# dusk-network/jubjub-schnorr

Hardware: AMD Instinct MI355X
Metric: Schnorr verifications/sec (higher is better)
Workload: dtype u32 limbs (29-bit), u64 accumulators

## Files before the change

### jubjub_schnorr_amd/csrc/ed29.h

```cpp
#pragma once
#include "fq29.h"

namespace jjs {

using fe_t = fe<1, 5>;

struct ext_pt {
    fe_n x, y, z, t;
};
struct niels_pt {
    fe_t ypx, ymx, z, t2d;
};

JJS_HD fe_n fe_n_one() { return fq_as<1, 2>(fq_one()); }
JJS_HD fe_n fe_n_zero() { return fq_as<1, 2>(fq_zero()); }

JJS_HD ext_pt ext_identity() {
    ext_pt p;
    p.x = fe_n_zero(); p.y = fe_n_one(); p.z = fe_n_one(); p.t = fe_n_zero();
    return p;
}
JJS_HD ext_pt ext_from_affine(const fe_n& u, const fe_n& v) {
    ext_pt p;
    p.x = u; p.y = v; p.z = fe_n_one(); p.t = fq_mul(u, v);
// ... 30 lines not shown
    ext_pt r;
    r.x = fq_mul_hot(e, f);
    r.z = fq_mul_hot(f, h);
    r.y = fq_mul_hot(h, g);
    if (need_t) r.t = fq_mul_hot(g, e); else r.t = fe_n_zero();
    return r;
}

JJS_HD ext_pt ext_add_niels(const ext_pt& p, const niels_pt& n, bool neg, bool need_t) {
    fe_t n_ymx = fq_select(neg, n.ypx, n.ymx);
    fe_t n_ypx = fq_select(neg, n.ymx, n.ypx);
    auto n_t2d = fq_select(neg, fq_neg(n.t2d), fq_as<2, 6>(n.t2d));
    fe_n a = fq_mul_hot(fq_sub(p.y, p.x), n_ymx);
    fe_n b = fq_mul_hot(fq_add(p.y, p.x), n_ypx);
    fe_n c = fq_mul_hot(p.t, n_t2d);
    auto d = fq_dbl(fq_mul_hot(p.z, n.z));
    auto e = fq_sub(b, a);
    auto f = fq_norm(fq_sub(d, c));
    auto g = fq_add(d, c);
    auto h = fq_norm(fq_add(b, a));
    ext_pt r;
    r.x = fq_mul_hot(e, f);
    r.z = fq_mul_hot(f, g);
    r.y = fq_mul_hot(g, h);
    if (need_t) r.t = fq_mul_hot(h, e); else r.t = fe_n_zero();
    return r;
}
JJS_HD ext_pt ext_add_affine_niels_signed(const ext_pt& p, const fe_t& n_ypx, const fe_t& n_ymx, const fe_t& n_t2d, bool neg,
                                          bool need_t) {
    fe_t s_ymx = fq_select(neg, n_ypx, n_ymx);
    fe_t s_ypx = fq_select(neg, n_ymx, n_ypx);
    auto s_t2d = fq_select(neg, fq_neg(n_t2d), fq_as<2, 6>(n_t2d));
    fe_n a = fq_mul_hot(fq_sub(p.y, p.x), s_ymx);
    fe_n b = fq_mul_hot(fq_add(p.y, p.x), s_ypx);
    fe_n c = fq_mul_hot(p.t, s_t2d);
    auto d = fq_dbl(p.z);
    auto e = fq_sub(b, a);
    auto f = fq_norm(fq_sub(d, c));
    auto g = fq_add(d, c);
    auto h = fq_norm(fq_add(b, a));
    ext_pt r;
    r.x = fq_mul_hot(e, f);
    r.z = fq_mul_hot(f, g);
    r.y = fq_mul_hot(g, h);
    if (need_t) r.t = fq_mul_hot(h, e); else r.t = fe_n_zero();
    return r;
}

JJS_HD ext_pt ext_add_affine_niels(const ext_pt& p, const fe_t& n_ypx, const fe_t& n_ymx, const fe_t& n_t2d,
                                   bool need_t) {
    return ext_add_affine_niels_signed(p, n_ypx, n_ymx, n_t2d, false, need_t);
}

JJS_HD bool ext_is_identity(const ext_pt& p) { return fq_is_zero(p.x) && fq_eq(p.y, p.z); }

JJS_HD bool affine_on_curve(const fe_n& u, const fe_n& v) {
    fe_n u2 = fq_sqr(u), v2 = fq_sqr(v);
    auto lhs = fq_sub(v2, u2);
    auto rhs = fq_norm(fq_add(fq_mul(fq_mul(u2, v2), fe_from_const<1, 1>(JJS_D)), fq_one()));
    return fq_eq(lhs, rhs);
}
JJS_HD bool affine_is_identity(const fe_n& u, const fe_n& v) { return fq_is_zero(u) && fq_eq(v, fq_one()); }

JJS_HD bool ext_eq_affine(const ext_pt& p, const fe_n& u, const fe_n& v) {
    return fq_eq(p.x, fq_mul(u, p.z)) && fq_eq(p.y, fq_mul(v, p.z));
}

}
```

### jubjub_schnorr_amd/csrc/fq29.h

```cpp
#pragma once
#include <stdint.h>

#if defined(__HIPCC__)
#include <hip/hip_runtime.h>
#define JJS_HD __host__ __device__ __forceinline__
#define JJS_CALL __host__ __device__ __attribute__((noinline))
#if defined(__HIP_DEVICE_COMPILE__)
#define JJS_CONST __constant__ const
#else
#define JJS_CONST static const
#endif
#else
#define JJS_HD inline __attribute__((always_inline))
#define JJS_CALL __attribute__((noinline))
#define JJS_CONST static const
#endif

namespace jjs {

#include "jjs_constants.inc"
#include "mont_asm.inc"

constexpr uint32_t MASK29 = 0x1fffffffu;

// ... 61 lines not shown
    for (int i = 0; i < 9; ++i) r.l[i] = a.l[i] + b.l[i];
    return r;
}
template <int L, int A>
JJS_HD fe<2 * L, 2 * A> fq_dbl(const fe<L, A>& a) {
    fe<2 * L, 2 * A> r;
#pragma unroll
    for (int i = 0; i < 9; ++i) r.l[i] = a.l[i] << 1;
    return r;
}
template <int La, int Aa, int Ab>
JJS_HD fe<La + 2, Aa + Ab + 1> fq_sub(const fe<La, Aa>& a, const fe<1, Ab>& b) {
    fe<La + 2, Aa + Ab + 1> r;
#pragma unroll
    for (int i = 0; i < 9; ++i) r.l[i] = a.l[i] + (subpad29(Ab + 1, i) - b.l[i]);
    return r;
}
template <int Ab>
JJS_HD fe<2, Ab + 1> fq_neg(const fe<1, Ab>& b) {
    fe<2, Ab + 1> r;
#pragma unroll
    for (int i = 0; i < 9; ++i) r.l[i] = subpad29(Ab + 1, i) - b.l[i];
    return r;
}
template <int L, int A>
JJS_HD fe<1, A> fq_norm(const fe<L, A>& a) {
    fe<1, A> r;
    uint32_t carry = 0;
#pragma unroll
    for (int i = 0; i < 8; ++i) {
        uint32_t t = a.l[i] + carry;
        r.l[i] = t & MASK29;
        carry = t >> 29;
    }
    r.l[8] = a.l[8] + carry;
    return r;
}
template <int A>
JJS_HD fe_n fq_reduce(const fe<1, A>& a) {
    static_assert(A <= 4, "fq_reduce handles values below 4q");
    fe_n t;
    int32_t borrow = 0;
#pragma unroll
    for (int i = 0; i < 9; ++i) {
        int32_t d = (int32_t)a.l[i] - (int32_t)kq29(2, i) + borrow;
        t.l[i] = (uint32_t)d & MASK29;
        borrow = d >> 29;
        if (i == 8) t.l[8] = (uint32_t)d;
    }
    bool neg = borrow < 0;
    fe_n r;
#pragma unroll
    for (int i = 0; i < 9; ++i) r.l[i] = neg ? a.l[i] : t.l[i];
    return r;
}
template <int L, int A>
JJS_HD fe<L, A> fq_select(bool c, const fe<L, A>& a, const fe<L, A>& b) {
    fe<L, A> r;
#pragma unroll
    for (int i = 0; i < 9; ++i) r.l[i] = c ? a.l[i] : b.l[i];
    return r;
}

JJS_HD int64_t mont_ashr29(int64_t v) {
    return v >> 29;
}

JJS_HD raw9 mont_mul_body(const uint32_t* a, const uint32_t* b) {
    int64_t m[9];
    raw9 r;
    int64_t acc = 0;
#pragma unroll
    for (int k = 0; k < 9; ++k) {
#pragma unroll
        for (int i = 0; i <= k; ++i) acc += (int64_t)((uint64_t)a[i] * b[k - i]);
#pragma unroll
        for (int i = 0; i < k; ++i) acc -= m[i] * (int64_t)q29(k - i);
        if (k < 8) {
            m[k] = acc & (int64_t)MASK29;
            acc = mont_ashr29(acc);
        } else {
            m[8] = (acc & (int64_t)MASK29) - ((int64_t)1 << 29);
            acc = mont_ashr29(acc - m[8]);
        }
    }
#pragma unroll
    for (int k = 9; k < 17; ++k) {
#pragma unroll
        for (int i = k - 8; i < 9; ++i) acc += (int64_t)((uint64_t)a[i] * b[k - i]);
#pragma unroll
        for (int i = k - 8; i < 9; ++i) acc -= m[i] * (int64_t)q29(k - i);
        r.l[k - 9] = (uint32_t)(acc & (int64_t)MASK29);
        acc = mont_ashr29(acc);
    }
    r.l[8] = (uint32_t)acc;
    return r;
}
JJS_HD raw9 mont_sqr_body(const uint32_t* a) {
    int64_t m[9];
    uint32_t a2[9];
#pragma unroll
    for (int i = 0; i < 9; ++i) a2[i] = a[i] << 1;
    raw9 r;
    int64_t acc = 0;
#pragma unroll
    for (int k = 0; k < 17; ++k) {
// ... 233 lines not shown
    fe_c r;
#pragma unroll
    for (int i = 0; i < 9; ++i) {
        int bit = 29 * i, w = bit >> 5, sh = bit & 31;
        uint64_t v = a.w[w];
        if (w + 1 < 8) v |= (uint64_t)a.w[w + 1] << 32;
        r.l[i] = (uint32_t)(v >> sh) & MASK29;
    }
    return r;
}
JJS_HD fe_n fq_from_words(const words8& a) { return fq_mul(words_to_limbs(a), fe_from_const<1, 1>(JJS_R2)); }

template <int L, int A>
JJS_HD fe_c fq_canon_limbs(const fe<L, A>& a) {
    fe_c one = fq_zero();
    one.l[0] = 1;
    fe_n y = fq_mul(fq_norm(a), one);
    bool is_q = true;
#pragma unroll
    for (int i = 0; i < 9; ++i) is_q = is_q && (y.l[i] == q29(i));
    fe_c r;
#pragma unroll
    for (int i = 0; i < 9; ++i) r.l[i] = is_q ? 0u : y.l[i];
    return r;
}
template <int L, int A>
JJS_HD words8 fq_to_words(const fe<L, A>& a) {
    fe_c c = fq_canon_limbs(a);
    words8 o;
#pragma unroll
    for (int w = 0; w < 8; ++w) {
        int bit = 32 * w, i = bit / 29, sh = bit - 29 * i;
        uint64_t v = (uint64_t)c.l[i] >> sh;
        int have = 29 - sh;
        v |= (uint64_t)c.l[i + 1] << have;
        if (have + 29 < 32 && i + 2 < 9) v |= (uint64_t)c.l[i + 2] << (have + 29);
        o.w[w] = (uint32_t)v;
    }
    return o;
}
template <int L, int A>
JJS_HD bool fq_is_zero(const fe<L, A>& a) {
    fe_c c = fq_canon_limbs(a);
    uint32_t x = 0;
#pragma unroll
    for (int i = 0; i < 9; ++i) x |= c.l[i];
    return x == 0;
}
template <int La, int Aa, int Ab>
JJS_HD bool fq_eq(const fe<La, Aa>& a, const fe<1, Ab>& b) {
    return fq_is_zero(fq_sub(a, b));
}

JJS_HD fe_n fq_pow_schedule(const fe_n& a, const uint32_t (*sched)[2], int steps, int trailing) {
    fe_n a2 = fq_sqr(a);
    fe_n a3 = fq_mul(a2, a), a5 = fq_mul(a3, a2), a7 = fq_mul(a5, a2);
    fe_n e = a;
    for (int st = 0; st < steps; ++st) {
        const uint32_t nsq = sched[st][0], dg = sched[st][1];
        if (st != 0)
            for (uint32_t j = 0; j < nsq; ++j) e = fq_sqr(e);
        const fe_n m = fq_select(dg == 1, a, fq_select(dg == 3, a3, fq_select(dg == 5, a5, a7)));
        e = (st == 0) ? m : fq_mul(e, m);
    }
    for (int j = 0; j < trailing; ++j) e = fq_sqr(e);
    return e;
}
}
```

### jubjub_schnorr_amd/csrc/jjs_constants.inc

```
#define JJS_MAX_HASH_INPUTS 16
#define JJS_Q29_0 0x00000001u
#define JJS_Q29_1 0x1ffffff8u
#define JJS_Q29_2 0x1f96ffbfu
#define JJS_Q29_3 0x1b4805ffu
#define JJS_Q29_4 0x1d80553bu
#define JJS_Q29_5 0x0c0404d0u
#define JJS_Q29_6 0x1520cce7u
#define JJS_Q29_7 0x0a6533afu
#define JJS_Q29_8 0x0073eda7u
JJS_CONST uint32_t JJS_Q_WORDS[8] = {0x00000001u, 0xffffffffu, 0xfffe5bfeu, 0x53bda402u, 0x09a1d805u, 0x3339d808u, 0x299d7d48u, 0x73eda753u};
JJS_CONST uint32_t JJS_QM2_WORDS[8] = {0xffffffffu, 0xfffffffeu, 0xfffe5bfeu, 0x53bda402u, 0x09a1d805u, 0x3339d808u, 0x299d7d48u, 0x73eda753u};
JJS_CONST uint32_t JJS_FR_WORDS[8] = {0xd6f72cb7u, 0xd0970e5eu, 0xccc81082u, 0xa6682093u, 0x01343b00u, 0x06673b01u, 0x6533afa9u, 0x0e7db4eau};
JJS_CONST uint32_t JJS_FR_R2_WORDS[8] = {0x95e57731u, 0x67719aa4u, 0x9ce3fc26u, 0x51b0cef0u, 0xc026e9a5u, 0x69dab7fau, 0x8d127688u, 0x04f6547bu};
#define JJS_FR_INV32 0xef788ef9u
JJS_CONST uint32_t JJS_R2[9] = {0x0a71b3c0u, 0x1d32207eu, 0x1663d999u, 0x1c5abc93u, 0x03b58c44u, 0x0be37438u, 0x0829f771u, 0x1660139eu, 0x0027fd91u};
JJS_CONST uint32_t JJS_ONE[9] = {0x1fffffbau, 0x0000022fu, 0x1cb61180u, 0x0a4e5c00u, 0x0ee8b1a2u, 0x16e6aedfu, 0x1907f8bbu, 0x0853ddf7u, 0x004d043fu};
JJS_CONST uint32_t JJS_D[9] = {0x0e9ed5e8u, 0x12245679u, 0x002d9f52u, 0x03bb3367u, 0x0d9bfb3du, 0x18ebb3ccu, 0x1c29ceccu, 0x0a7b6020u, 0x0020d725u};
JJS_CONST uint32_t JJS_D2[9] = {0x1d3dabd0u, 0x0448acf2u, 0x005b3ea5u, 0x077666ceu, 0x1b37f67au, 0x11d76798u, 0x18539d99u, 0x14f6c041u, 0x0041ae4au};
JJS_CONST uint32_t JJS_G[2][9] = {{0x0f8e352bu, 0x0d898cfcu, 0x1acf8b86u, 0x11cbaed5u, 0x11f53f06u, 0x1e102b0eu, 0x1a54d9c6u, 0x143eceffu, 0x006815d6u}, {0x1ffffb09u, 0x000027b7u, 0x09503dc0u, 0x0d6a3610u, 0x07d8d3d7u, 0x180c16bcu, 0x1a26af41u, 0x038c62dfu, 0x006f1642u}};
JJS_CONST uint32_t JJS_GN[2][9] = {{0x187d023du, 0x137e7289u, 0x0690434eu, 0x1f76361du, 0x00cee7a6u, 0x0f6ffe89u, 0x0eae76dcu, 0x0b002f63u, 0x001b3c2eu}, {0x0d19dfe5u, 0x1ba2bfe4u, 0x0aa87077u, 0x0a3c12aeu, 0x0f209d38u, 0x03331d80u, 0x05e964c7u, 0x046d436du, 0x00027722u}};
JJS_CONST uint32_t JJS_DOUBLE_TAG_WORDS[8] = {0x4844424cu, 0x4a4a5343u, 0x00000000u, 0x00000000u, 0x00000000u, 0x00000000u, 0x00000000u, 0x00000000u};
JJS_CONST uint32_t JJS_SPONGE_TAG[JJS_MAX_HASH_INPUTS + 1][9] = {
  {0x00000000u, 0x00000000u, 0x00000000u, 0x00000000u, 0x00000000u, 0x00000000u, 0x00000000u, 0x00000000u, 0x00000000u},
  {0x0505ee08u, 0x1a263c20u, 0x0be84b8bu, 0x14a02c49u, 0x01c71b32u, 0x0119871du, 0x0e158ab3u, 0x1ae4f29eu, 0x002534dfu},
  {0x1b0be909u, 0x1f0bd4a7u, 0x15c76ef6u, 0x19aa6651u, 0x03d277dau, 0x02c51eb8u, 0x131e6edfu, 0x1c823839u, 0x0028ae1cu},
  {0x0fc46418u, 0x0273db7eu, 0x16529079u, 0x104dd318u, 0x168e8637u, 0x026f5725u, 0x1c808eacu, 0x029e0e17u, 0x003fedbdu},
  {0x0357c163u, 0x10043808u, 0x19bdf7a6u, 0x0d30d38fu, 0x12e5297bu, 0x1c58dc5fu, 0x0ba83205u, 0x06d45679u, 0x00090830u},
  {0x0262554eu, 0x06977c58u, 0x1cc4c932u, 0x13bcc122u, 0x0d7d7321u, 0x16c6f8cdu, 0x0c42072du, 0x0a7ba9d5u, 0x00467f10u},
  {0x16ed364au, 0x0b0ae88eu, 0x1bd377f9u, 0x1bebcca6u, 0x0fbf0111u, 0x0eacca90u, 0x174be582u, 0x0d8cb0dfu, 0x006048a8u},
  {0x1648d83cu, 0x1c96a336u, 0x13f93121u, 0x0404c2c5u, 0x12088053u, 0x05063ca4u, 0x1387a958u, 0x0e2ca8b5u, 0x000dc63bu},
  {0x1f8df888u, 0x05a7ef5au, 0x1e8dea4fu, 0x04cf9c40u, 0x03a338cdu, 0x11ce25feu, 0x08f757fcu, 0x197c5746u, 0x00448b3du},
  {0x18861d85u, 0x0bfc90f3u, 0x01a0c7f1u, 0x0b8f8540u, 0x061d8364u, 0x17492b24u, 0x1f89fbceu, 0x03e0f6e4u, 0x002d13cau},
  {0x0f24fc1du, 0x17584430u, 0x197f7236u, 0x1bad9229u, 0x17ce7252u, 0x12745987u, 0x119f85a5u, 0x0365f792u, 0x00419641u},
  {0x0ad4ee1du, 0x1c33dd77u, 0x03cea63au, 0x0090b229u, 0x1eff0500u, 0x1ae3d4a9u, 0x0e58224eu, 0x1ba57ecau, 0x00131c30u},
  {0x0047e885u, 0x12b591deu, 0x09f50887u, 0x0c3877f6u, 0x01adcabbu, 0x00dcbf79u, 0x0ac6f554u, 0x0bcc64deu, 0x0062115cu},
  {0x18868630u, 0x0c3e88d9u, 0x0d12f54du, 0x062083b4u, 0x00efbe4eu, 0x1c915ba8u, 0x11f90d73u, 0x1200490cu, 0x00205cd9u},
  {0x109c52e0u, 0x100352e0u, 0x0d1863ecu, 0x0f9203ccu, 0x08db7deau, 0x1ea7d49cu, 0x0641cbbeu, 0x1693107au, 0x00056607u},
  {0x07380761u, 0x0379c563u, 0x10c89db4u, 0x0924fcebu, 0x0cf29ce1u, 0x1bfecb19u, 0x1a3ca913u, 0x12d81574u, 0x0008852cu},
  {0x0137f8a1u, 0x135b43b9u, 0x1a25c48fu, 0x04e620e0u, 0x0f670a49u, 0x190a832du, 0x1c3afc44u, 0x0c7a93dbu, 0x0026b4abu},
};
JJS_CONST uint32_t JJS_PAIR_L1[2][9] = {{0x1632f828u, 0x1cd998edu, 0x06ef42eau, 0x18522084u, 0x12362748u, 0x02a698c9u, 0x1b29c579u, 0x021b0691u, 0x003c41f3u}, {0x1b06fde4u, 0x137cdc5cu, 0x1714b9b2u, 0x065d7f7du, 0x140f3e68u, 0x08fb5d4bu, 0x18ad857au, 0x02b255c2u, 0x005ac97bu}};
JJS_CONST uint32_t JJS_PAIR_NEG_L2[9] = {0x0ec609f6u, 0x0fa98aa5u, 0x012a02e2u, 0x17e06bfeu, 0x14bb44c6u, 0x0c66138cu, 0x166a4edbu, 0x0ffd0b0au, 0x0050cfe0u};
JJS_CONST uint32_t JJS_PAIR_B[9] = {0x002c2b67u, 0x1e9ea4c8u, 0x07b6263fu, 0x1afbd911u, 0x133cdbc5u, 0x16559828u, 0x1a61d3c3u, 0x10975a2au, 0x00520471u};
JJS_CONST uint32_t JJS_PAIR_EXP_WORDS[8] = {0xe0000000u, 0xdfffffffu, 0x5fffcb7fu, 0xaa77b480u, 0x01343b00u, 0x06673b01u, 0x6533afa9u, 0x0e7db4eau};
#define JJS_PAIR_SW_STEPS 57
#define JJS_PAIR_SW_TRAILING 29
JJS_CONST uint32_t JJS_PAIR_SW[JJS_PAIR_SW_STEPS][2] = {{3, 7}, {5, 7}, {2, 3}, {3, 3}, {3, 3}, {2, 1}, {5, 7}, {4, 5}, {4, 3}, {5, 5}, {4, 3}, {5, 7}, {4, 5}, {3, 7}, {3, 5}, {2, 1}, {3, 1}, {7, 3}, {4, 3}, {5, 7}, {5, 7}, {3, 3}, {8, 1}, {8, 1}, {4, 3}, {2, 1}, {7, 7}, {3, 3}, {11, 5}, {4, 5}, {5, 7}, {4, 7}, {3, 5}, {3, 5}, {3, 1}, {11, 5}, {3, 7}, {3, 7}, {3, 7}, {3, 7}, {2, 3}, {5, 5}, {3, 5}, {3, 7}, {3, 7}, {2, 3}, {4, 7}, {3, 7}, {3, 7}, {3, 7}, {3, 7}, {3, 7}, {3, 7}, {3, 7}, {3, 7}, {3, 7}, {2, 3}};
#define JJS_INV_SW_STEPS 68
#define JJS_INV_SW_TRAILING 0
JJS_CONST uint32_t JJS_INV_SW[JJS_INV_SW_STEPS][2] = {{3, 7}, {5, 7}, {2, 3}, {3, 3}, {3, 3}, {2, 1}, {5, 7}, {4, 5}, {4, 3}, {5, 5}, {4, 3}, {5, 7}, {4, 5}, {3, 7}, {3, 5}, {2, 1}, {3, 1}, {7, 3}, {4, 3}, {5, 7}, {5, 7}, {3, 3}, {8, 1}, {8, 1}, {4, 3}, {2, 1}, {7, 7}, {3, 3}, {11, 5}, {4, 5}, {5, 7}, {4, 7}, {3, 5}, {3, 5}, {3, 1}, {11, 5}, {3, 7}, {3, 7}, {3, 7}, {3, 7}, {2, 3}, {5, 5}, {3, 5}, {3, 7}, {3, 7}, {2, 3}, {4, 7}, {3, 7}, {3, 7}, {3, 7}, {3, 7}, {3, 7}, {3, 7}, {3, 7}, {3, 7}, {3, 7}, {3, 5}, {3, 7}, {3, 7}, {3, 7}, {3, 7}, {3, 7}, {3, 7}, {3, 7}, {3, 7}, {3, 7}, {3, 7}, {1, 1}};
#define JJS_SQRT_SW_STEPS 57
#define JJS_SQRT_SW_TRAILING 0
JJS_CONST uint32_t JJS_SQRT_SW[JJS_SQRT_SW_STEPS][2] = {{3, 7}, {5, 7}, {2, 3}, {3, 3}, {3, 3}, {2, 1}, {5, 7}, {4, 5}, {4, 3}, {5, 5}, {4, 3}, {5, 7}, {4, 5}, {3, 7}, {3, 5}, {2, 1}, {3, 1}, {7, 3}, {4, 3}, {5, 7}, {5, 7}, {3, 3}, {8, 1}, {8, 1}, {4, 3}, {2, 1}, {7, 7}, {3, 3}, {11, 5}, {4, 5}, {5, 7}, {4, 7}, {3, 5}, {3, 5}, {3, 1}, {11, 5}, {3, 7}, {3, 7}, {3, 7}, {3, 7}, {2, 3}, {5, 5}, {3, 5}, {3, 7}, {3, 7}, {2, 3}, {4, 7}, {3, 7}, {3, 7}, {3, 7}, {3, 7}, {3, 7}, {3, 7}, {3, 7}, {3, 7}, {3, 7}, {1, 1}};
JJS_CONST uint32_t JJS_DLOG_BASES[7][9] = {{0x1e643334u, 0x16481b3cu, 0x1b429d12u, 0x177f9dadu, 0x144a8d18u, 0x0d45bdd8u, 0x04734720u, 0x08d7bfb9u, 0x0036d431u}, {0x015b5931u, 0x170bf111u, 0x0fdc692cu, 0x1da57375u, 0x1cd8fb0cu, 0x082b2e9eu, 0x11dae58du, 0x1c3e92cdu, 0x007386deu}, {0x046746cau, 0x011b8fe2u, 0x1ba33a6du, 0x176e1524u, 0x09d99e75u, 0x154d7d8eu, 0x00d23d31u, 0x1df2d37eu, 0x000963afu}, {0x1e643334u, 0x16481b3cu, 0x1b429d12u, 0x177f9dadu, 0x144a8d18u, 0x0d45bdd8u, 0x04734720u, 0x08d7bfb9u, 0x0036d431u}, {0x065b9ba7u, 0x16d68576u, 0x182b2c2au, 0x14d5af02u, 0x07140888u, 0x1362f1d7u, 0x08c77bb2u, 0x1cb1a9c5u, 0x00094bf1u}, {0x1abc62ceu, 0x0fbddb01u, 0x140b0090u, 0x03bc5521u, 0x11f8af58u, 0x1881ae47u, 0x11d5d43eu, 0x0a2d9980u, 0x005fe400u}, {0x04fbdc84u, 0x10c8e2ffu, 0x041d8af4u, 0x1a3da377u, 0x19ceef70u, 0x002b6e41u, 0x0034a007u, 0x1c185b28u, 0x0007ee60u}};
#define JJS_DLOG_HASH_MULT 1u
#define JJS_DLOG_HASH_SHIFT 0
JJS_CONST uint32_t JJS_ROOT_OF_UNITY[9] = {0x01c8cd27u, 0x158d8d27u, 0x19006c0du, 0x09177006u, 0x1b40635eu, 0x01d0b1cau, 0x0d517805u, 0x04859aa2u, 0x002c4064u};
JJS_CONST uint32_t JJS_RC[340][9] = {
  {0x00acd34au, 0x1735f45au, 0x138d6d99u, 0x0ed55d98u, 0x1ca62dc6u, 0x10ba9671u, 0x10435733u, 0x033b644du, 0x004aa8c7u},
  {0x14ffba26u, 0x1ba29e52u, 0x177f0b64u, 0x00b3510cu, 0x127726cfu, 0x1857d2a8u, 0x1e3d168au, 0x15e4d101u, 0x000f1ecau},
  {0x10544837u, 0x105827efu, 0x084c6e15u, 0x0e8aac41u, 0x0ae02b0fu, 0x18ebde5au, 0x0fafaf7cu, 0x083d3281u, 0x0034fd73u},
  {0x0344bf7fu, 0x0a46646au, 0x1730014du, 0x12e0ba85u, 0x02e3906cu, 0x05e7a406u, 0x17f2dc8bu, 0x1945722eu, 0x003a6ecfu},
  {0x1fd22f28u, 0x045b2ea8u, 0x17a649b2u, 0x0f9d7504u, 0x11961944u, 0x1660a34bu, 0x0a6a6237u, 0x193bc629u, 0x0021ffc7u},
  {0x1d29e5b8u, 0x06cae729u, 0x151ba656u, 0x1ac9f0b1u, 0x1b3a5e51u, 0x0d4ca236u, 0x1207ea27u, 0x1d21fa02u, 0x0022dd1fu},
  {0x12400ff9u, 0x0035d81du, 0x03b62299u, 0x025d538au, 0x08e06dddu, 0x1bbf452cu, 0x094dfd08u, 0x00285210u, 0x00308fabu},
  {0x1d184e77u, 0x1592ad1fu, 0x16661d64u, 0x1fe21660u, 0x1bfeebb3u, 0x0b7e4ad3u, 0x17ca297au, 0x15006fa8u, 0x001db197u},
  {0x1ddad3c4u, 0x13a1d246u, 0x071c897bu, 0x164f9a39u, 0x0689f7a5u, 0x080f8889u, 0x135aee92u, 0x03a580b3u, 0x006f4972u},
  {0x0d6eb0dbu, 0x058fde5bu, 0x1499b97cu, 0x0f49db3bu, 0x0ed02c77u, 0x0cd55fdeu, 0x029ef2fbu, 0x1f5282afu, 0x002a2cdcu},
  {0x1ab8ab5fu, 0x027938ecu, 0x0c556f7eu, 0x09fbfaf8u, 0x0ae0ef37u, 0x19cb8097u, 0x0358d657u, 0x12a3f282u, 0x002ebee0u},
  {0x12dd5a05u, 0x1eba6f91u, 0x00b2d3d3u, 0x0aa6ae2cu, 0x13721dbbu, 0x1619de12u, 0x0b03bb30u, 0x1947db06u, 0x000b396bu},
  {0x1f8c17c0u, 0x01352a93u, 0x09e2ed99u, 0x07dac2cdu, 0x0d3aedbeu, 0x053f5f63u, 0x1b33c7e7u, 0x10c2ba42u, 0x0057396bu},
// ... 473 lines not shown
```

### jubjub_schnorr_amd/csrc/key_tables.h

```cpp
#pragma once
#include "verify_core.h"
#include "decode.h"
#include "ed29_quad.h"

namespace jjs {

constexpr int KT_WINDOW_NARROW = 5, KT_WINDOW_WIDE = 6;
constexpr uint32_t KT_WIDE_MULTIPLICITY = 128;
JJS_HD constexpr int kt_positions(int w) { return (252 + w) / w; }
JJS_HD constexpr int kt_entries(int w) { return (1 << (w - 1)) + 1; }
JJS_HD constexpr int kt_table_words(int w) { return kt_entries(w) * ENTRY_WORDS; }
constexpr int KT_MAX_POSITIONS = kt_positions(KT_WINDOW_NARROW);
static_assert(KT_WINDOW_NARROW >= 4 && KT_WINDOW_WIDE <= 6 && KT_WINDOW_NARROW < KT_WINDOW_WIDE, "digit extraction assumes a digit spans at most two words");
constexpr uint32_t KT_MIN_MULTIPLICITY = 16;
constexpr uint32_t KT_MAX_PROBES = 128;
constexpr uint32_t KT_KEY_MALFORMED = 1, KT_KEY_VALID = 2;
constexpr int KT_BASE_WORDS = 36;
JJS_HD constexpr size_t kt_max(size_t a, size_t b) { return a > b ? a : b; }
JJS_HD constexpr size_t kt_base_words_for_keys(size_t narrow, size_t wide) {
    return kt_max(narrow * kt_positions(KT_WINDOW_NARROW), wide * kt_positions(KT_WINDOW_WIDE)) * KT_BASE_WORDS;
}
JJS_HD constexpr size_t kt_table_words_for_keys(size_t narrow, size_t wide) {
    return kt_max(narrow * kt_positions(KT_WINDOW_NARROW) * kt_table_words(KT_WINDOW_NARROW),
                  wide * kt_positions(KT_WINDOW_WIDE) * kt_table_words(KT_WINDOW_WIDE));
// ... 269 lines not shown
        const fe_n u = fq_mul_hot(e.ypx, zi), v = fq_mul_hot(e.ymx, zi);
        niels_pt n;
        n.ypx = fq_as<1, 5>(fq_norm(fq_add(v, u)));
        n.ymx = fq_norm(fq_sub(v, u));
        n.z = fq_as<1, 5>(fq_one());
        n.t2d = fq_as<1, 5>(fq_mul_hot(fq_mul_hot(u, v), fe_from_const<1, 1>(JJS_D2)));
        store_niels(tab + j * ENTRY_WORDS, n);
        e = below;
    }
}
JJS_HD void kt_table_lane(const key_column& C, uint32_t id, uint32_t pos, int w) {
    const uint32_t pi = kt_pool(C, id);
    kt_build_table(kt_table(C, pi, pos, w), kt_load_ext(kt_base(C, pi, pos, w)), kt_entries(w));
}

JJS_HD constexpr uint32_t kt_recode_word(int w, int word) {
    uint32_t v = 0;
    for (int i = 0; i < kt_positions(w) - 1; ++i) {
        const int bit = w * i + w - 1;
        if ((bit >> 5) == word) v |= 1u << (bit & 31);
    }
    return v;
}
JJS_HD words8 kt_recode(const words8& s, int w) {
    constexpr uint32_t KN[8] = {kt_recode_word(KT_WINDOW_NARROW, 0), kt_recode_word(KT_WINDOW_NARROW, 1), kt_recode_word(KT_WINDOW_NARROW, 2),
                                kt_recode_word(KT_WINDOW_NARROW, 3), kt_recode_word(KT_WINDOW_NARROW, 4), kt_recode_word(KT_WINDOW_NARROW, 5),
                                kt_recode_word(KT_WINDOW_NARROW, 6), kt_recode_word(KT_WINDOW_NARROW, 7)};
    constexpr uint32_t KW[8] = {kt_recode_word(KT_WINDOW_WIDE, 0), kt_recode_word(KT_WINDOW_WIDE, 1), kt_recode_word(KT_WINDOW_WIDE, 2),
                                kt_recode_word(KT_WINDOW_WIDE, 3), kt_recode_word(KT_WINDOW_WIDE, 4), kt_recode_word(KT_WINDOW_WIDE, 5),
                                kt_recode_word(KT_WINDOW_WIDE, 6), kt_recode_word(KT_WINDOW_WIDE, 7)};
    const bool wide = w == KT_WINDOW_WIDE;
    words8 r;
    uint64_t carry = 0;
#pragma unroll
    for (int i = 0; i < 8; ++i) {
        const uint64_t t = (uint64_t)s.w[i] + (wide ? KW[i] : KN[i]) + carry;
        r.w[i] = (uint32_t)t;
        carry = t >> 32;
    }
    return r;
}
JJS_HD void kt_load_affine(const uint32_t* src, fe_t& ypx, fe_t& ymx, fe_t& t2d) {
    const u32x4* p = reinterpret_cast<const u32x4*>(src);
    uint32_t w[ENTRY_WORDS];
#pragma unroll
    for (int i = 0; i < ENTRY_WORDS / 4; ++i) {
        if (i == 5) continue;
        const u32x4 v = p[i];
        w[4 * i] = v.x; w[4 * i + 1] = v.y; w[4 * i + 2] = v.z; w[4 * i + 3] = v.w;
    }
#pragma unroll
    for (int i = 0; i < 9; ++i) { ypx.l[i] = w[i]; ymx.l[i] = w[9 + i]; t2d.l[i] = w[27 + i]; }
}
JJS_HD ext_pt kt_add_digit(const ext_pt& acc, const uint32_t* tab, const words8& sc, int pos, int w) {
    const int bit = w * pos, wi = bit >> 5, sh = bit & 31;
    uint32_t v = word_at(sc, wi) >> sh;
    if (sh + w > 32) v |= word_at(sc, wi + 1 > 7 ? 7 : wi + 1) << (32 - sh);
    const uint32_t raw = v & ((1u << w) - 1u);
    const bool top = pos == kt_positions(w) - 1;
    const int d = top ? (int)(word_at(sc, wi) >> sh) : (int)raw - (1 << (w - 1));
    const bool neg = d < 0;
    uint32_t idx = (uint32_t)(neg ? -d : d);
    idx = idx >= (uint32_t)kt_entries(w) ? (uint32_t)kt_entries(w) - 1u : idx;
    fe_t ypx, ymx, t2d;
    kt_load_affine(tab + idx * ENTRY_WORDS, ypx, ymx, t2d);
    return ext_add_affine_niels_signed(acc, ypx, ymx, t2d, neg, true);
}
JJS_HD ext_pt kt_add_scalar(ext_pt acc, const key_column& C, uint32_t id, const words8& s, int w) {
    const words8 sc = kt_recode(s, w);
    const uint32_t pi = kt_pool(C, id);
    for (int pos = kt_positions(w) - 1; pos >= 0; --pos) acc = kt_add_digit(acc, kt_table(C, pi, (uint32_t)pos, w), sc, pos, w);
    return acc;
}
JJS_HD constexpr int kt_challenge_positions(int w) { return kt_positions(w) - (w == KT_WINDOW_WIDE ? 1 : 0); }
static_assert(KT_WINDOW_WIDE * (kt_positions(KT_WINDOW_WIDE) - 1) >= 252 && KT_WINDOW_NARROW * (kt_positions(KT_WINDOW_NARROW) - 1) <= 250,
              "which top positions a 250-bit scalar leaves empty");
JJS_HD ext_pt kt_add_challenge(ext_pt acc, const key_column& C, uint32_t id, const words8& c, int w) {
    const words8 sc = kt_recode(c, w);
    const uint32_t pi = kt_pool(C, id);
    for (int pos = kt_challenge_positions(w) - 1; pos >= 0; --pos) acc = kt_add_digit(acc, kt_table(C, pi, (uint32_t)pos, w), sc, pos, w);
    return acc;
}

JJS_HD uint32_t kt_finish_item(const verify_params& P, const key_params& K, uint64_t item, const prep_record& r) {
    const int w = (int)*P.key_flag;
    const words8 u = load_words(P.u, item);
    bool keys_valid = true, keys_malformed = false, eq_ok = true;
    for (uint32_t e = 0; e < P.n_eq; ++e) {
        const eq_desc& E = P.eq[e];
        ext_pt acc = ext_identity();
        {
            const key_column C = kt_col(K, E.pk_col);
            const uint32_t id = C.keyid[item], f = C.key_flags[id];
            keys_valid = keys_valid && (f & KT_KEY_VALID) != 0;
            keys_malformed = keys_malformed || (f & KT_KEY_MALFORMED) != 0;
            acc = kt_add_challenge(acc, C, id, r.c, w);
        }
        if (E.comb) {
            acc = add_comb(acc, E.comb, u, JJS_SKIP(P, 16u));
        } else {
            const key_column C = kt_col(K, E.gen_col);
            const uint32_t id = C.keyid[item], f = C.key_flags[id];
            keys_valid = keys_valid && (f & KT_KEY_VALID) != 0;
            keys_malformed = keys_malformed || (f & KT_KEY_MALFORMED) != 0;
            acc = kt_add_scalar(acc, C, id, u, w);
        }
        const fe_n ru = load_fq(E.r, item), rv = load_fq(E.r, item, 32);
        eq_ok = ext_eq_affine(acc, ru, rv) && eq_ok;
    }
    if (r.malformed || keys_malformed || !words_lt(u, JJS_FR_WORDS)) return ST_MALFORMED;
    if (!r.valid || !keys_valid) return ST_INVALID_POINT;
    if (JJS_SKIP(P, 1u)) return eq_ok ? ST_OK : ST_INVALID_SIGNATURE;
    return eq_ok ? ST_OK : ST_PENDING_EQ_FAILED;
}

}
```

### jubjub_schnorr_amd/csrc/verify_core.h

```cpp
#pragma once
#include <cmath>

#include "ed29.h"
#include "hades29.h"
#include "fq_inv.h"

namespace jjs {

enum : uint32_t { ST_OK = 0, ST_INVALID_POINT = 1, ST_INVALID_SIGNATURE = 2, ST_MALFORMED = 3 };
enum : uint32_t { ST_PENDING_EQ_FAILED = 4, ST_PENDING_EQ_HELD = 5 };

struct fe_src {
    const uint8_t* base;
    uint32_t stride;
    uint32_t off;
};
struct eq_desc {
    const uint32_t* comb;
    fe_src gen;
    fe_src pk;
    fe_src r;
    int32_t pk_col, gen_col;
};
struct verify_params {
// ... 434 lines not shown
        }
#pragma unroll
        for (int i = 0; i < 4; ++i) {
            const uint32_t a = m0[i], b = t1[i];
            t0[i] = swap ? b : a;
            t1[i] = swap ? a : b;
        }
        neg = swap ? !neg : neg;
    }
    half_scalars h;
#pragma unroll
    for (int i = 0; i < 4; ++i) { h.a.w[i] = r1[i]; h.b.w[i] = t1[i]; }
    h.b_neg = neg;
    return h;
}

JJS_HD bool is_torsion_free_by_order(const fe_n& u, const fe_n& v) {
    ext_pt p = ext_from_affine(u, v);
    niels_pt n = to_niels(p);
    ext_pt acc = p;
    for (int i = 250; i >= 0; --i) {
        bool bit = (JJS_FR_WORDS[i >> 5] >> (i & 31)) & 1;
        acc = ext_double(acc, bit);
        if (bit) acc = ext_add_affine_niels(acc, n.ypx, n.ymx, n.t2d, false);
    }
    return ext_is_identity(acc);
}

JJS_HD bool pairing_is_trivial(const fe_n& px, const fe_n& py, const fe_n& pz) {
    auto opv = fq_add(pz, py);
    auto omv = fq_sub(pz, py);
    fe_n w = fq_mul(omv, px);
    fe_n x = fq_mul(opv, px);
    fe_n oz = fq_mul(opv, pz);
    fe_n xw[2] = {x, w};
    auto l1 = fq_norm(fq_add(oz, fq_dot_const<2, 2>(JJS_PAIR_L1, xw)));
    auto l2 = fq_norm(fq_add(oz, fq_mul(x, fe_from_const<1, 1>(JJS_PAIR_NEG_L2))));
    auto vv = fq_norm(fq_sub(x, w));
    fe_n a = fq_mul(fq_sqr(l1), l2);
    a = fq_sqr(fq_mul(a, fq_sqr(vv)));
    fe_n y = fq_mul(fq_mul(x, w), fe_from_const<1, 1>(JJS_PAIR_B));
    fe_n y2 = fq_sqr(y);
    fe_n y7 = fq_mul(fq_mul(fq_sqr(y2), y2), y);
    fe_n g = fq_mul(a, y7);
    fe_n e = fq_pow_schedule(g, JJS_PAIR_SW, JJS_PAIR_SW_STEPS, JJS_PAIR_SW_TRAILING);
    return fq_eq(e, fq_one());
}
JJS_HD bool is_torsion_free(const fe_n& u, const fe_n& v) { return pairing_is_trivial(u, v, fe_n_one()); }

JJS_HD bool point_on_curve_not_identity(const fe_n& u, const fe_n& v) {
    return affine_on_curve(u, v) && !affine_is_identity(u, v);
}

JJS_HD ext_pt add_comb_range(ext_pt acc, const uint32_t* comb, const words8& k, int lo, int hi, bool t_last,
                             bool one_entry = false) {
    for (int i = lo; i < hi; ++i) {
        constexpr int per_word = 32 / COMB_BITS;
        uint32_t digit = (word_at(k, i / per_word) >> ((i % per_word) * COMB_BITS)) & (uint32_t)(COMB_ENTRIES - 1);
        digit = one_entry ? (digit & 255u) : digit;
        const u32x4* p = reinterpret_cast<const u32x4*>(comb + ((size_t)i * COMB_ENTRIES + digit) * COMB_ENTRY_WORDS);
        uint32_t w[COMB_ENTRY_WORDS];
#pragma unroll
        for (int k4 = 0; k4 < COMB_ENTRY_WORDS / 4; ++k4) { u32x4 v = p[k4]; w[4 * k4] = v.x; w[4 * k4 + 1] = v.y; w[4 * k4 + 2] = v.z; w[4 * k4 + 3] = v.w; }
        fe_t ypx, ymx, t2d;
#pragma unroll
        for (int j = 0; j < 9; ++j) { ypx.l[j] = w[j]; ymx.l[j] = w[9 + j]; t2d.l[j] = w[18 + j]; }
        acc = ext_add_affine_niels(acc, ypx, ymx, t2d, t_last || i != hi - 1);
    }
    return acc;
}
JJS_HD ext_pt add_comb(ext_pt acc, const uint32_t* comb, const words8& k, bool one_entry = false) {
    return add_comb_range(acc, comb, k, 0, COMB_WINDOWS, false, one_entry);
}
JJS_HD words8 widen128(const u128w& x) {
    words8 r;
#pragma unroll
    for (int i = 0; i < 8; ++i) r.w[i] = i < 4 ? x.w[i] : 0u;
    return r;
}
JJS_HD words8 recode_signed4_128(const u128w& s) {
    words8 r;
    uint64_t carry = 0;
#pragma unroll
    for (int i = 0; i < 8; ++i) {
        uint64_t t = (uint64_t)(i < 4 ? s.w[i] : 0u) + (i < 3 ? 0x88888888u : (i == 3 ? 0x08888888u : 0u)) + carry;
        r.w[i] = (uint32_t)t;
        carry = t >> 32;
    }
    return r;
}

JJS_HD words8 half_scalar_times_u(const half_scalars& h, const words8& u) {
    words8 r2;
#pragma unroll
    for (int i = 0; i < 8; ++i) r2.w[i] = JJS_FR_R2_WORDS[i];
    words8 w = fr_mont_mul(fr_mont_mul(widen128(h.b), r2), u);
    uint32_t nz = 0, borrow = 0;
    words8 n;
#pragma unroll
    for (int i = 0; i < 8; ++i) {
        nz |= w.w[i];
        uint64_t d = (uint64_t)JJS_FR_WORDS[i] - w.w[i] - borrow;
        n.w[i] = (uint32_t)d;
        borrow = (uint32_t)(d >> 63);
    }
    return select_words(h.b_neg && nz != 0, n, w);
}

JJS_HD bool check_equation(const eq_desc& E, uint64_t item, uint32_t* ws, const words8& u, const words8& c,
                           const half_scalars& h, const uint32_t* shared_tab = nullptr) {
    const bool one_entry = shared_tab != nullptr;
    const bool fixed = (E.comb != nullptr);
#pragma unroll 1
    for (int t = 0; t < 2; ++t) {
        const fe_src& src = (t == 0) ? E.pk : (fixed ? E.r : E.gen);
        fe_n pu = load_fq(src, item), pv = load_fq(src, item, 32);
        build_point_table(ws + t * TABLE_WORDS, pu, pv);
    }
    words8 s0, s1, w;
// ... 209 lines not shown
```

Measured before the change: 124.3 million.

## Seed key-table accumulator from first digit and fuse final add with equality check

The challenge multiplication now initializes the accumulator directly from the top table digit, converted from affine Niels form, instead of adding it to the identity. The last addition of the verification equation is merged with the affine comparison, so the final x/z and y/z products are replaced by cross-multiplying the candidate R coordinates against the unnormalized add terms. This removes one full point addition and several field multiplications per equation. It adds a new wide reduction helper and a looser equality test that assumes bounded input ranges.

After: 124.2 million. Within noise of the previous version (-0.1%).

```diff
diff --git a/jubjub_schnorr_amd/csrc/ed29.h b/jubjub_schnorr_amd/csrc/ed29.h
--- a/jubjub_schnorr_amd/csrc/ed29.h
+++ b/jubjub_schnorr_amd/csrc/ed29.h
@@ -106,6 +106,36 @@
     return ext_add_affine_niels_signed(p, n_ypx, n_ymx, n_t2d, false, need_t);
 }
 
+JJS_HD ext_pt ext_from_affine_niels_signed(const fe_t& n_ypx, const fe_t& n_ymx, const fe_t& n_t2d, bool neg) {
+    fe_t s_ymx = fq_select(neg, n_ypx, n_ymx);
+    fe_t s_ypx = fq_select(neg, n_ymx, n_ypx);
+    auto s_t2d = fq_select(neg, fq_neg(n_t2d), fq_as<2, 6>(n_t2d));
+    ext_pt r;
+    r.x = fq_reduce_wide(fq_norm(fq_sub(s_ypx, s_ymx)));
+    r.y = fq_reduce_wide(fq_norm(fq_add(s_ypx, s_ymx)));
+    r.z = fq_norm(fq_dbl(fq_one()));
+    r.t = fq_mul(s_t2d, fe_from_const<1, 1>(JJS_D_INV));
+    return r;
+}
+
+JJS_HD bool ext_add_affine_niels_signed_eq(const ext_pt& p, const fe_t& n_ypx, const fe_t& n_ymx, const fe_t& n_t2d, bool neg,
+                                           const fe_c& u, const fe_c& v) {
+    fe_t s_ymx = fq_select(neg, n_ypx, n_ymx);
+    fe_t s_ypx = fq_select(neg, n_ymx, n_ypx);
+    auto s_t2d = fq_select(neg, fq_neg(n_t2d), fq_as<2, 6>(n_t2d));
+    fe_n a = fq_mul_hot(fq_sub(p.y, p.x), s_ymx);
+    fe_n b = fq_mul_hot(fq_add(p.y, p.x), s_ypx);
+    fe_n c = fq_mul_hot(p.t, s_t2d);
+    auto d = fq_dbl(p.z);
+    auto e = fq_sub(b, a);
+    auto f = fq_norm(fq_sub(d, c));
+    auto g = fq_add(d, c);
+    auto h = fq_add(b, a);
+    const bool x_ok = fq_plain_eq(fq_canon_limbs(e), fq_mul(u, g));
+    const bool y_ok = fq_plain_eq(fq_canon_limbs(h), fq_mul(v, f));
+    return x_ok && y_ok;
+}
+
 JJS_HD bool ext_is_identity(const ext_pt& p) { return fq_is_zero(p.x) && fq_eq(p.y, p.z); }
 
 JJS_HD bool affine_on_curve(const fe_n& u, const fe_n& v) {
diff --git a/jubjub_schnorr_amd/csrc/fq29.h b/jubjub_schnorr_amd/csrc/fq29.h
--- a/jubjub_schnorr_amd/csrc/fq29.h
+++ b/jubjub_schnorr_amd/csrc/fq29.h
@@ -137,6 +137,21 @@
     fe_n r;
 #pragma unroll
     for (int i = 0; i < 9; ++i) r.l[i] = neg ? a.l[i] : t.l[i];
+    return r;
+}
+template <int A>
+JJS_HD fe_n fq_reduce_wide(const fe<1, A>& a) {
+    static_assert(A <= 16, "fq_reduce_wide handles values below 16q");
+    const uint32_t k = a.l[8] / (q29(8) + 1u);
+    fe_n r;
+    int64_t borrow = 0;
+#pragma unroll
+    for (int i = 0; i < 9; ++i) {
+        const int64_t d = (int64_t)a.l[i] - (int64_t)((uint64_t)k * q29(i)) + borrow;
+        r.l[i] = (uint32_t)d & MASK29;
+        borrow = d >> 29;
+        if (i == 8) r.l[8] = (uint32_t)d;
+    }
     return r;
 }
 template <int L, int A>
@@ -476,6 +491,14 @@
     return fq_is_zero(fq_sub(a, b));
 }
 
+JJS_HD bool fq_plain_eq(const fe_c& c, const fe_n& t) {
+    const auto d = fq_norm(fq_sub(c, t));
+    bool is2 = true, is3 = true;
+#pragma unroll
+    for (int i = 0; i < 9; ++i) { is2 = is2 && d.l[i] == kq29(2, i); is3 = is3 && d.l[i] == kq29(3, i); }
+    return is2 || is3;
+}
+
 JJS_HD fe_n fq_pow_schedule(const fe_n& a, const uint32_t (*sched)[2], int steps, int trailing) {
     fe_n a2 = fq_sqr(a);
     fe_n a3 = fq_mul(a2, a), a5 = fq_mul(a3, a2), a7 = fq_mul(a5, a2);
diff --git a/jubjub_schnorr_amd/csrc/jjs_constants.inc b/jubjub_schnorr_amd/csrc/jjs_constants.inc
--- a/jubjub_schnorr_amd/csrc/jjs_constants.inc
+++ b/jubjub_schnorr_amd/csrc/jjs_constants.inc
@@ -17,6 +17,7 @@
 JJS_CONST uint32_t JJS_ONE[9] = {0x1fffffbau, 0x0000022fu, 0x1cb61180u, 0x0a4e5c00u, 0x0ee8b1a2u, 0x16e6aedfu, 0x1907f8bbu, 0x0853ddf7u, 0x004d043fu};
 JJS_CONST uint32_t JJS_D[9] = {0x0e9ed5e8u, 0x12245679u, 0x002d9f52u, 0x03bb3367u, 0x0d9bfb3du, 0x18ebb3ccu, 0x1c29ceccu, 0x0a7b6020u, 0x0020d725u};
 JJS_CONST uint32_t JJS_D2[9] = {0x1d3dabd0u, 0x0448acf2u, 0x005b3ea5u, 0x077666ceu, 0x1b37f67au, 0x11d76798u, 0x18539d99u, 0x14f6c041u, 0x0041ae4au};
+JJS_CONST uint32_t JJS_D_INV[9] = {0x066666aeu, 0x1ffffdc3u, 0x0908547fu, 0x148b4732u, 0x004b09f0u, 0x0f8625a2u, 0x1592e8b6u, 0x1b814187u, 0x006bab32u};
 JJS_CONST uint32_t JJS_G[2][9] = {{0x0f8e352bu, 0x0d898cfcu, 0x1acf8b86u, 0x11cbaed5u, 0x11f53f06u, 0x1e102b0eu, 0x1a54d9c6u, 0x143eceffu, 0x006815d6u}, {0x1ffffb09u, 0x000027b7u, 0x09503dc0u, 0x0d6a3610u, 0x07d8d3d7u, 0x180c16bcu, 0x1a26af41u, 0x038c62dfu, 0x006f1642u}};
 JJS_CONST uint32_t JJS_GN[2][9] = {{0x187d023du, 0x137e7289u, 0x0690434eu, 0x1f76361du, 0x00cee7a6u, 0x0f6ffe89u, 0x0eae76dcu, 0x0b002f63u, 0x001b3c2eu}, {0x0d19dfe5u, 0x1ba2bfe4u, 0x0aa87077u, 0x0a3c12aeu, 0x0f209d38u, 0x03331d80u, 0x05e964c7u, 0x046d436du, 0x00027722u}};
 JJS_CONST uint32_t JJS_DOUBLE_TAG_WORDS[8] = {0x4844424cu, 0x4a4a5343u, 0x00000000u, 0x00000000u, 0x00000000u, 0x00000000u, 0x00000000u, 0x00000000u};
diff --git a/jubjub_schnorr_amd/csrc/key_tables.h b/jubjub_schnorr_amd/csrc/key_tables.h
--- a/jubjub_schnorr_amd/csrc/key_tables.h
+++ b/jubjub_schnorr_amd/csrc/key_tables.h
@@ -345,7 +345,7 @@
 #pragma unroll
     for (int i = 0; i < 9; ++i) { ypx.l[i] = w[i]; ymx.l[i] = w[9 + i]; t2d.l[i] = w[27 + i]; }
 }
-JJS_HD ext_pt kt_add_digit(const ext_pt& acc, const uint32_t* tab, const words8& sc, int pos, int w) {
+JJS_HD bool kt_load_digit(const uint32_t* tab, const words8& sc, int pos, int w, fe_t& ypx, fe_t& ymx, fe_t& t2d) {
     const int bit = w * pos, wi = bit >> 5, sh = bit & 31;
     uint32_t v = word_at(sc, wi) >> sh;
     if (sh + w > 32) v |= word_at(sc, wi + 1 > 7 ? 7 : wi + 1) << (32 - sh);
@@ -355,9 +355,18 @@
     const bool neg = d < 0;
     uint32_t idx = (uint32_t)(neg ? -d : d);
     idx = idx >= (uint32_t)kt_entries(w) ? (uint32_t)kt_entries(w) - 1u : idx;
+    kt_load_affine(tab + idx * ENTRY_WORDS, ypx, ymx, t2d);
+    return neg;
+}
+JJS_HD ext_pt kt_add_digit(const ext_pt& acc, const uint32_t* tab, const words8& sc, int pos, int w) {
     fe_t ypx, ymx, t2d;
-    kt_load_affine(tab + idx * ENTRY_WORDS, ypx, ymx, t2d);
+    const bool neg = kt_load_digit(tab, sc, pos, w, ypx, ymx, t2d);
     return ext_add_affine_niels_signed(acc, ypx, ymx, t2d, neg, true);
+}
+JJS_HD ext_pt kt_from_digit(const uint32_t* tab, const words8& sc, int pos, int w) {
+    fe_t ypx, ymx, t2d;
+    const bool neg = kt_load_digit(tab, sc, pos, w, ypx, ymx, t2d);
+    return ext_from_affine_niels_signed(ypx, ymx, t2d, neg);
 }
 JJS_HD ext_pt kt_add_scalar(ext_pt acc, const key_column& C, uint32_t id, const words8& s, int w) {
     const words8 sc = kt_recode(s, w);
@@ -372,6 +381,14 @@
     const words8 sc = kt_recode(c, w);
     const uint32_t pi = kt_pool(C, id);
     for (int pos = kt_challenge_positions(w) - 1; pos >= 0; --pos) acc = kt_add_digit(acc, kt_table(C, pi, (uint32_t)pos, w), sc, pos, w);
+    return acc;
+}
+JJS_HD ext_pt kt_mul_challenge(const key_column& C, uint32_t id, const words8& c, int w) {
+    const words8 sc = kt_recode(c, w);
+    const uint32_t pi = kt_pool(C, id);
+    const int top = kt_challenge_positions(w) - 1;
+    ext_pt acc = kt_from_digit(kt_table(C, pi, (uint32_t)top, w), sc, top, w);
+    for (int pos = top - 1; pos >= 0; --pos) acc = kt_add_digit(acc, kt_table(C, pi, (uint32_t)pos, w), sc, pos, w);
     return acc;
 }
 
@@ -381,25 +398,31 @@
     bool keys_valid = true, keys_malformed = false, eq_ok = true;
     for (uint32_t e = 0; e < P.n_eq; ++e) {
         const eq_desc& E = P.eq[e];
-        ext_pt acc = ext_identity();
+        ext_pt acc;
         {
             const key_column C = kt_col(K, E.pk_col);
             const uint32_t id = C.keyid[item], f = C.key_flags[id];
             keys_valid = keys_valid && (f & KT_KEY_VALID) != 0;
             keys_malformed = keys_malformed || (f & KT_KEY_MALFORMED) != 0;
-            acc = kt_add_challenge(acc, C, id, r.c, w);
+            acc = kt_mul_challenge(C, id, r.c, w);
         }
+        fe_t ypx, ymx, t2d;
+        bool neg = false;
         if (E.comb) {
-            acc = add_comb(acc, E.comb, u, JJS_SKIP(P, 16u));
+            acc = add_comb_range(acc, E.comb, u, 0, COMB_WINDOWS - 1, true, JJS_SKIP(P, 16u));
+            comb_load(E.comb, u, COMB_WINDOWS - 1, JJS_SKIP(P, 16u), ypx, ymx, t2d);
         } else {
             const key_column C = kt_col(K, E.gen_col);
             const uint32_t id = C.keyid[item], f = C.key_flags[id];
             keys_valid = keys_valid && (f & KT_KEY_VALID) != 0;
             keys_malformed = keys_malformed || (f & KT_KEY_MALFORMED) != 0;
-            acc = kt_add_scalar(acc, C, id, u, w);
+            const words8 sc = kt_recode(u, w);
+            const uint32_t pi = kt_pool(C, id);
+            for (int pos = kt_positions(w) - 1; pos >= 1; --pos) acc = kt_add_digit(acc, kt_table(C, pi, (uint32_t)pos, w), sc, pos, w);
+            neg = kt_load_digit(kt_table(C, pi, 0u, w), sc, 0, w, ypx, ymx, t2d);
         }
-        const fe_n ru = load_fq(E.r, item), rv = load_fq(E.r, item, 32);
-        eq_ok = ext_eq_affine(acc, ru, rv) && eq_ok;
+        const fe_c ru = words_to_limbs(load_words(E.r, item)), rv = words_to_limbs(load_words(E.r, item, 32));
+        eq_ok = ext_add_affine_niels_signed_eq(acc, ypx, ymx, t2d, neg, ru, rv) && eq_ok;
     }
     if (r.malformed || keys_malformed || !words_lt(u, JJS_FR_WORDS)) return ST_MALFORMED;
     if (!r.valid || !keys_valid) return ST_INVALID_POINT;
diff --git a/jubjub_schnorr_amd/csrc/verify_core.h b/jubjub_schnorr_amd/csrc/verify_core.h
--- a/jubjub_schnorr_amd/csrc/verify_core.h
+++ b/jubjub_schnorr_amd/csrc/verify_core.h
@@ -510,19 +510,22 @@
     return affine_on_curve(u, v) && !affine_is_identity(u, v);
 }
 
+JJS_HD void comb_load(const uint32_t* comb, const words8& k, int i, bool one_entry, fe_t& ypx, fe_t& ymx, fe_t& t2d) {
+    constexpr int per_word = 32 / COMB_BITS;
+    uint32_t digit = (word_at(k, i / per_word) >> ((i % per_word) * COMB_BITS)) & (uint32_t)(COMB_ENTRIES - 1);
+    digit = one_entry ? (digit & 255u) : digit;
+    const u32x4* p = reinterpret_cast<const u32x4*>(comb + ((size_t)i * COMB_ENTRIES + digit) * COMB_ENTRY_WORDS);
+    uint32_t w[COMB_ENTRY_WORDS];
+#pragma unroll
+    for (int k4 = 0; k4 < COMB_ENTRY_WORDS / 4; ++k4) { u32x4 v = p[k4]; w[4 * k4] = v.x; w[4 * k4 + 1] = v.y; w[4 * k4 + 2] = v.z; w[4 * k4 + 3] = v.w; }
+#pragma unroll
+    for (int j = 0; j < 9; ++j) { ypx.l[j] = w[j]; ymx.l[j] = w[9 + j]; t2d.l[j] = w[18 + j]; }
+}
 JJS_HD ext_pt add_comb_range(ext_pt acc, const uint32_t* comb, const words8& k, int lo, int hi, bool t_last,
                              bool one_entry = false) {
     for (int i = lo; i < hi; ++i) {
-        constexpr int per_word = 32 / COMB_BITS;
-        uint32_t digit = (word_at(k, i / per_word) >> ((i % per_word) * COMB_BITS)) & (uint32_t)(COMB_ENTRIES - 1);
-        digit = one_entry ? (digit & 255u) : digit;
-        const u32x4* p = reinterpret_cast<const u32x4*>(comb + ((size_t)i * COMB_ENTRIES + digit) * COMB_ENTRY_WORDS);
-        uint32_t w[COMB_ENTRY_WORDS];
-#pragma unroll
-        for (int k4 = 0; k4 < COMB_ENTRY_WORDS / 4; ++k4) { u32x4 v = p[k4]; w[4 * k4] = v.x; w[4 * k4 + 1] = v.y; w[4 * k4 + 2] = v.z; w[4 * k4 + 3] = v.w; }
         fe_t ypx, ymx, t2d;
-#pragma unroll
-        for (int j = 0; j < 9; ++j) { ypx.l[j] = w[j]; ymx.l[j] = w[9 + j]; t2d.l[j] = w[18 + j]; }
+        comb_load(comb, k, i, one_entry, ypx, ymx, t2d);
         acc = ext_add_affine_niels(acc, ypx, ymx, t2d, t_last || i != hi - 1);
     }
     return acc;
```
